# bhavyageethika/multimodal_autonomous_driving_perception_and_planning

Hardware: AMD Instinct MI355X
Metric: end-to-end frames/sec (1280x720 synthetic) (higher is better)
Workload: dtype f64; 1 GPU; config4: 64 stream(s)/GPU x 1-frame window per step, 1280x720, simulated detection + IoU tracker + 6-state KF + 21-candidate planner, one launch per step, up to 4 consecutive steps in flight; streams_per_gpu=64, window=1, graph=False, taggers=False, allgather_track_tables=False, fused_step=True, overlapped_steps=4, steps_per_library_call=8, parallelism=stream-sharded x1

## Files before the change

multimodal_autonomous_driving_perception_and_planning_amd/csrc/common.h:

```cpp
#pragma once
#include <hip/hip_runtime.h>

#include <cstdarg>
#include <cstdio>
#include <vector>

#include "avhot.h"

struct PlannerTables;

struct av_ctx {
    int device = -1;
    int n_cus = 256;
    hipStream_t side = nullptr;
    hipEvent_t ev_fork = nullptr, ev_join = nullptr;
    bool planner_ready = false;
    av_planner_cfg pcfg{};
    int n_points = 0, n_lat = 0, n_cand = 0;
    double* d_ptab = nullptr;
    double* d_cdf = nullptr;
    void* d_simtab = nullptr;
    std::vector<hipGraphExec_t> graphs;
    void* lane = nullptr;
    void* yolo = nullptr;
};

void av_set_error(const char* fmt, ...);

#define AV_HIP(expr)                                                                          \
    do {                                                                                      \
        hipError_t e_ = (expr);                                                               \
        if (e_ != hipSuccess) {                                                               \
            av_set_error("%s:%d: %s -> %s", __FILE__, __LINE__, #expr, hipGetErrorString(e_)); \
            return AV_EHIP;                                                                   \
        }                                                                                     \
    } while (0)

#define AV_REQUIRE(cond, code, ...)   \
    do {                              \
        if (!(cond)) {                \
            av_set_error(__VA_ARGS__); \
            return (code);            \
        }                             \
    } while (0)

#define AV_LAUNCH_CHECK()                                                                \
    do {                                                                                 \
        hipError_t e_ = hipGetLastError();                                               \
        if (e_ != hipSuccess) {                                                          \
            av_set_error("%s:%d: kernel launch -> %s", __FILE__, __LINE__, hipGetErrorString(e_)); \
            return AV_EHIP;                                                              \
        }                                                                                \
    } while (0)

static inline hipStream_t as_stream(av_stream_t s) { return reinterpret_cast<hipStream_t>(s); }

__device__ __forceinline__ int lane_id() { return (int)(threadIdx.x & 63); }

__device__ __forceinline__ double wave_sum(double v) {
#pragma unroll
    for (int off = 32; off > 0; off >>= 1) v += __shfl_xor(v, off, 64);
    return v;
}
template <int CTRL, int ROW_MASK = 0xF, bool BOUND = true>
__device__ __forceinline__ double dpp_mov_f64(double v) {
    const int lo = __double2loint(v), hi = __double2hiint(v);
    const int nlo = __builtin_amdgcn_update_dpp(0, lo, CTRL, ROW_MASK, 0xF, BOUND);
    const int nhi = __builtin_amdgcn_update_dpp(0, hi, CTRL, ROW_MASK, 0xF, BOUND);
    return __hiloint2double(nhi, nlo);
}
__device__ __forceinline__ double readlane_f64(double v, int l) {
    return __hiloint2double(__builtin_amdgcn_readlane(__double2hiint(v), l),
// ... 98 lines not shown
```

multimodal_autonomous_driving_perception_and_planning_amd/csrc/planner.hip:

```cpp
#include "common.h"

#include <cmath>



namespace {

struct PlanParams {
    int n, n_lat, C;
    double dt, H;
    double w_lat, w_vel, w_acc, w_curv;
    const double *t, *alpha, *q, *dtd, *lat;
    double atq[20];
};

static const double ATAN_Q[20] = {
    -0x1.5555555555549p-2, 0x1.99999999979b9p-3,  -0x1.24924923e22b4p-3, 0x1.c71c718e5a102p-4,
    -0x1.745d120df88fbp-4, 0x1.3b1362fc35ab5p-4,  -0x1.110deef367776p-4, 0x1.e1b3c8d50e91fp-5,
    -0x1.ae2c7119eb922p-5, 0x1.81fdd2525246ap-5,  -0x1.56daf4786fd80p-5, 0x1.2575526b2309ap-5,
    -0x1.d168e01adf666p-6, 0x1.462cc26bda000p-6,  -0x1.8055065b73333p-7, 0x1.693bd6b79999ap-8,
    -0x1.fdf4e15cccccdp-10, 0x1.f224118000000p-12, -0x1.2568700000000p-14, 0x1.2ed799999999ap-18,
};

__device__ __forceinline__ double atan2_fast(double y, double x, const double (&Q)[20]) {
// ... 15 lines not shown
    a = x < 0.0 ? 3.141592653589793 - a : a;
    return __builtin_copysign(a, y);
}

__host__ __device__ inline int even_up(int v) { return (v + 1) & ~1; }

__host__ __device__ inline size_t plan_lds_doubles(int G, int n, int C, int NW = 4) {
    return (size_t)G * 3 * n * 2 + even_up(G * 3 * 3) + (size_t)G * 8 + (size_t)3 * even_up(G * C) + (size_t)NW * n * 6;
}

__device__ __forceinline__ void wave_lds_fence() {
    __builtin_amdgcn_fence(__ATOMIC_RELEASE, "wavefront", "local");
    __builtin_amdgcn_wave_barrier();
    __builtin_amdgcn_fence(__ATOMIC_ACQUIRE, "wavefront", "local");
}

template <int G, int NW>
__device__ __forceinline__ void plan_block(const PlanParams& p, int f0, int n_states, const double* __restrict__ state,
                                           const double* __restrict__ ref, int n_ref, const double* __restrict__ obs, int n_obs,
                                           double* __restrict__ wp, double* __restrict__ cost, int32_t* __restrict__ order, double* sm) {
    const int n = p.n, C = p.C;
    double* vs = sm;
    double* base = vs + (size_t)G * 3 * n * 2;
    double* trig = base + even_up(G * 3 * 3);
    double* costs = trig + G * 8;
    double* stage_all = costs + 3 * even_up(G * C);
    const int CS = even_up(G * C);

    const int tid = threadIdx.x, lane = tid & 63, wid = tid >> 6;
    double* stage = stage_all + (size_t)wid * n * 6;
    constexpr int P = G * 3;
    static_assert(NW >= 2, "the heading terms take the last wave");

    auto bcast = [&](double x, int i) {
        const unsigned lo = (unsigned)__builtin_amdgcn_readlane((int)(unsigned)__double_as_longlong(x), i);
        const unsigned hi = (unsigned)__builtin_amdgcn_readlane((int)(unsigned)((unsigned long long)__double_as_longlong(x) >> 32), i);
        return __longlong_as_double((long long)(((unsigned long long)hi << 32) | lo));
    };
    auto terms = [&](double v0, double dv, int i, double& v, double& vdt, double& velt, double& acct) {
        v = v0 + dv * p.alpha[i];
        vdt = v * p.dt;
        const double e = v - 10.0;
        velt = p.w_vel * (e * e);
        acct = 0.0;
        if (i > 0) {
            const double vp = v0 + dv * p.alpha[i - 1];
            const double a = (v - vp) / p.dtd[i];
            acct = p.w_acc * (a * a);
        }
    };
    auto cost_chains = [&](double velt, double acct, unsigned long long hasm, double* b) {
        double sv = 0.0;
#pragma unroll
        for (int i = 0; i < 64; ++i)
            if (i < n) sv = sv + bcast(velt, i);
        double run = sv, sa = 0.0;
#pragma unroll
        for (int i = 1; i < 64; ++i)
            if (i < n && ((hasm >> i) & 1ull)) {
                const double term = bcast(acct, i);
                run = run + term, sa = sa + term;
            }
        if (lane == 0) b[0] = sv, b[1] = sa, b[2] = run;
    };

    const bool fast = n <= 64 && P <= NW;
    double k_velt = 0.0, k_acct = 0.0;
    unsigned long long k_has = 0;
    bool k_live = false;
    if (fast) {
        if (wid < P) {
            const int g = wid / 3, k = wid - g * 3, f = f0 + g;
            if (f < n_states) {
                const double v0 = state[(size_t)f * 4 + 3];
                const double vt = 8.0 + 2.0 * (double)k;
                const double dv = vt - v0;
                double* o = vs + ((size_t)(g * 3 + k) * n) * 2;
                double v = 0.0, vdt = 0.0;
                bool has = false;
                if (lane < n) terms(v0, dv, lane, v, vdt, k_velt, k_acct), has = lane > 0 && p.dtd[lane] > 0.0;
                k_has = __ballot(has), k_live = true;
                double sacc = 0.0, my_s = 0.0;
#pragma unroll
                for (int i = 1; i < 64; ++i)
                    if (i < n) {
                        sacc = sacc + bcast(vdt, i);
                        my_s = lane == i ? sacc : my_s;
                    }
                if (lane < n) o[2 * lane] = v, o[2 * lane + 1] = my_s;
            }
        }
    } else {
        for (int pr = wid; pr < P; pr += NW) {
            const int g = pr / 3, k = pr - g * 3, f = f0 + g;
            if (f >= n_states) continue;
            const double v0 = state[(size_t)f * 4 + 3];
            const double vt = 8.0 + 2.0 * (double)k;
            const double dv = vt - v0;
            double* o = vs + ((size_t)(g * 3 + k) * n) * 2;
            double* b = base + (g * 3 + k) * 3;
            double* tv = stage;
            for (int i = lane; i < n; i += 64) {
                double v, vdt, velt, acct;
                terms(v0, dv, i, v, vdt, velt, acct);
                o[2 * i] = v, tv[i] = vdt, tv[n + i] = velt, tv[2 * n + i] = acct;
            }
            wave_lds_fence();
            if (lane == 0) {
                double sacc = 0.0, sv = 0.0;
                o[1] = 0.0;
                sv = sv + tv[n];
                for (int i = 1; i < n; ++i) {
                    sacc = sacc + tv[i];
                    o[2 * i + 1] = sacc;
                    sv = sv + tv[n + i];
// ... 594 lines not shown
```

multimodal_autonomous_driving_perception_and_planning_amd/csrc/step.hip:

```cpp
#define AVHOT_DEVICE_ONLY
#include "simdet.hip"
#include "tracker.hip"
#include "kf.hip"
#include "planner.hip"
#undef AVHOT_DEVICE_ONLY

namespace {

struct StepArgs {
    int S, h, w, dcap, tcap;
    av_tracker_cfg tcfg;
    av_kf_cfg kcfg;
    PlanParams pp;
    int32_t* frame_count; const SimRow* tab; const double* cdf;
    int32_t *det_n, *det_box, *det_cls; double* det_conf; int32_t* det_status;
    unsigned char* trk_state; av_track_row* snap; int32_t* snap_n; int32_t* det2trk;
    const double* z; double *kf_state, *vstate, *plan_state;
    double *wp, *cost; int32_t* order;
    uint8_t* wire; int stream0, frame0;
    int* flags; int seq, spin, fence, stage_off;
};

constexpr int STEP_NW = 8;

// ... 12 lines not shown
        t = n;
    }
};

__device__ void StepClock::start(const StepArgs& a, int role) {
    on = a.flags && (a.fence & 8) && threadIdx.x == 0;
    if (!on) return;
    acc = reinterpret_cast<unsigned long long*>(a.flags + flag_stats(a.S)) + role * 16;
    t = __builtin_amdgcn_s_memrealtime();
    atomicAdd(acc + 15, 1ull);
}

__device__ __forceinline__ bool seq_enter(const StepArgs& a, int slot, int* go) {
    if (threadIdx.x == 0) {
        int ok = 0;
        int* const counter = a.flags + 32 * slot;
        int* const fault = a.flags + flag_fault(a.S);
        const int want = a.seq, spin = a.spin;
        for (int n = 0; n <= spin; ++n) {
            if ((int)((unsigned)__hip_atomic_load(counter, __ATOMIC_RELAXED, __HIP_MEMORY_SCOPE_AGENT) - (unsigned)want) >= 0) { ok = 1; break; }
            if ((n & 255) == 255 && __hip_atomic_load(fault, __ATOMIC_RELAXED, __HIP_MEMORY_SCOPE_AGENT) != 0) break;
        }
        if (!ok) atomicOr(a.flags + flag_fault(a.S), 1);
        if (ok && (a.fence & 8) && a.seq != 0) {
            const unsigned long long tp = __hip_atomic_load(reinterpret_cast<unsigned long long*>(a.flags + 32 * slot + 2), __ATOMIC_RELAXED,
                                                            __HIP_MEMORY_SCOPE_AGENT);
            const unsigned long long now = __builtin_amdgcn_s_memrealtime();
            unsigned long long* acc = reinterpret_cast<unsigned long long*>(a.flags + flag_stats(a.S)) + (slot & 1) * 16;
            if (now > tp) atomicAdd(acc + 8, now - tp), atomicAdd(acc + 9, 1ull);
        }
        *go = ok;
    }
    __syncthreads();
    if (!*go) return false;
    if (a.fence & 1) __builtin_amdgcn_fence(__ATOMIC_ACQUIRE, "agent");
    return true;
}
__device__ __forceinline__ void seq_leave(const StepArgs& a, int slot) {
    if (a.fence & 2) __builtin_amdgcn_fence(__ATOMIC_RELEASE, "agent");
    if (a.fence & 8)
        __hip_atomic_store(reinterpret_cast<unsigned long long*>(a.flags + 32 * slot + 2), __builtin_amdgcn_s_memrealtime(), __ATOMIC_RELAXED,
                           __HIP_MEMORY_SCOPE_AGENT);
    __hip_atomic_store(a.flags + 32 * slot, (int)((unsigned)a.seq + 1u), __ATOMIC_RELAXED, __HIP_MEMORY_SCOPE_AGENT);
}
__device__ __forceinline__ void fetch_record(const void* src, void* dst_lds, int n8, int first, int end, bool coherent) {
    unsigned long long* g = const_cast<unsigned long long*>(reinterpret_cast<const unsigned long long*>(src));
    unsigned long long* l = reinterpret_cast<unsigned long long*>(dst_lds);
    if ((int)threadIdx.x < first || (int)threadIdx.x >= end) return;
    for (int i = (int)threadIdx.x - first; i < n8; i += end - first)
        l[i] = coherent ? __hip_atomic_load(g + i, __ATOMIC_RELAXED, __HIP_MEMORY_SCOPE_AGENT) : g[i];
}

template <int PW>
__global__ void __launch_bounds__(PW * 64) hot_step_kernel(StepArgs a) {
    extern __shared__ __attribute__((aligned(16))) unsigned char smem[];
    __shared__ int go, fc_stage;
    __shared__ __attribute__((aligned(16))) double kf_stage[AV_KF_STATE_DOUBLES + 2];
    __shared__ __attribute__((aligned(16))) int d_box[8 * 4];
    __shared__ __attribute__((aligned(16))) double d_conf[8], d_area[8], z_stage[4];
    __shared__ int d_cls[8], d_n[1];
    const int tid = threadIdx.x;
    const bool seq = a.flags != nullptr;
    if ((int)blockIdx.x < a.S) {
        if (PW > STEP_NW && tid >= STEP_NW * 64) return;
        const int s = blockIdx.x;
        StepClock ck;
        ck.start(a, 0);
        int fc_before = 0;
        if (tid == 0) {
            fc_before = seq ? (int)((unsigned)a.flags[flag_base(a.S) + s] + (unsigned)a.seq) : a.frame_count[s];
            fc_stage = fc_before;
            simdet_frame<true>(0, 0, 0, a.h, a.w, a.dcap, &fc_stage, a.tab, a.cdf, d_n, d_box, d_cls, d_conf,
                               a.det_status ? a.det_status + s : nullptr);
            for (int i = 0; i < a.dcap; ++i)
                d_area[i] = (double)(d_box[4 * i + 2] - d_box[4 * i]) * (double)(d_box[4 * i + 3] - d_box[4 * i + 1]);
        }
        ck.mark(0);
        if (seq && !seq_enter(a, 2 * s, &go)) return;
        ck.mark(1);
        unsigned char* stage = smem + a.stage_off;
        int fc0 = 0;
        if (seq && tid == 0) fc0 = __hip_atomic_load(a.frame_count + s, __ATOMIC_RELAXED, __HIP_MEMORY_SCOPE_AGENT);
        fetch_record(a.trk_state + (size_t)s * state_bytes(a.tcap, a.tcfg.trajectory_length), stage,
                     (HDR_INTS * 4 + a.tcap * (int)sizeof(av_track_row)) / 8, 64, STEP_NW * 64, seq);
        if (tid == 0) {
            if (seq) {
                if (fc0 != fc_before) atomicOr(a.flags + flag_fault(a.S), 2);
                __hip_atomic_store(a.frame_count + s, fc_stage, __ATOMIC_RELAXED, __HIP_MEMORY_SCOPE_AGENT);
            } else {
                a.frame_count[s] = fc_stage;
            }
        }
        if (seq) __builtin_amdgcn_s_waitcnt(0x0F70);
        __syncthreads();
        ck.mark(2);
        if (tid < a.dcap) {
            reinterpret_cast<int4*>(a.det_box)[(size_t)s * a.dcap + tid] = reinterpret_cast<const int4*>(d_box)[tid];
            a.det_cls[(size_t)s * a.dcap + tid] = d_cls[tid];
            a.det_conf[(size_t)s * a.dcap + tid] = d_conf[tid];
            if (tid == 0) a.det_n[s] = d_n[0];
        }
        tracker_body<false, 8, STEP_NW>(a.tcfg, 1, a.dcap, d_n, d_box, d_cls, d_conf, a.tcap, a.trk_state, a.snap, a.snap_n,
                                        a.det2trk, 1, s, smem, 0xFEDCBA9876543210ull, stage, seq, 0,
                                        seq ? a.flags + 32 * (2 * s) : nullptr, (int)((unsigned)a.seq + 1u), (a.fence & 8) != 0, d_area);
        ck.mark(3);
        if (a.wire) {
            __syncthreads();
// ... 1 lines not shown
                wire_put(a.wire + (size_t)s * (AV_WIRE_HDR_BYTES + (size_t)a.tcap * AV_WIRE_ROW_BYTES), tid, a.snap_n[s], a.tcap,
                         a.snap + (size_t)s * a.tcap, a.stream0 + s, a.frame0 + fc_stage);
        }
    } else {
        const int s = blockIdx.x - a.S;
        StepClock ck;
        ck.start(a, 1);
        if (tid < 4) z_stage[tid] = a.z[(size_t)s * 4 + tid];
        if (seq && !seq_enter(a, 2 * s + 1, &go)) return;
        ck.mark(1);
        if (tid < 64) {
            double* rec = a.kf_state + (size_t)s * AV_KF_STATE_DOUBLES;
            fetch_record(rec, kf_stage, AV_KF_STATE_DOUBLES, 0, 64, seq);
            __builtin_amdgcn_fence(__ATOMIC_RELEASE, "workgroup", "local");
            __builtin_amdgcn_wave_barrier();
            __builtin_amdgcn_fence(__ATOMIC_ACQUIRE, "workgroup", "local");
            ck.mark(2);
            const double* z = z_stage;
            double *vs = a.vstate + (size_t)s * AV_VSTATE_DOUBLES, *ps = a.plan_state + (size_t)s * 4;
            const bool separable = kf_axis_body(a.kcfg, 1, z, nullptr, kf_stage, vs, ps, 0, tid);
            if (!separable && tid == 0) kf_dense_stream_lds(a.kcfg, 0, 1, z, nullptr, kf_stage, vs, ps);
            __builtin_amdgcn_fence(__ATOMIC_RELEASE, "workgroup", "local");
            __builtin_amdgcn_wave_barrier();
            __builtin_amdgcn_fence(__ATOMIC_ACQUIRE, "workgroup", "local");
            if (tid < AV_KF_STATE_DOUBLES) {
                if (seq)
                    __hip_atomic_store(reinterpret_cast<unsigned long long*>(rec) + tid, (unsigned long long)__double_as_longlong(kf_stage[tid]),
                                       __ATOMIC_RELAXED, __HIP_MEMORY_SCOPE_AGENT);
                else
                    rec[tid] = kf_stage[tid];
            }
        }
        ck.mark(3);
        if (seq && tid < 64) {
            __builtin_amdgcn_s_waitcnt(0x0F70);
            if (tid == 0) seq_leave(a, 2 * s + 1);
        }
        ck.mark(4);
        __syncthreads();
        plan_block<1, PW>(a.pp, s, a.S, a.plan_state, nullptr, 0, nullptr, 0, a.wp, a.cost, a.order, reinterpret_cast<double*>(smem));
        ck.mark(6);
    }
}

}

static size_t hot_step_tracker_lds(int dcap, int tcap, int& stage_off) {
    static_assert(STEP_NW == 8, "tracker_lds_bytes sizes the replica kernel's eight column waves");
    const size_t lds_t = (tracker_lds_bytes(tcap, dcap, 1, true, 0) + 15) & ~size_t(15);
    stage_off = (int)lds_t;
    return lds_t + HDR_INTS * 4 + (size_t)tcap * sizeof(av_track_row);
}

static size_t hot_step_static_lds(const void* kernel) {
    hipFuncAttributes fa{};
    return hipFuncGetAttributes(&fa, kernel) == hipSuccess ? (size_t)fa.sharedSizeBytes : (size_t)16384;
}

static int hot_step_shape(const av_ctx* ctx, int n_streams, size_t lds_t, int depth, size_t& lds_out, int& pw_out) {
    static const size_t lds_static16 = hot_step_static_lds(reinterpret_cast<const void*>(hot_step_kernel<16>));
    static const size_t lds_static8 = hot_step_static_lds(reinterpret_cast<const void*>(hot_step_kernel<8>));
    const char* pwe = getenv("AVHOT_STEP_PW");
    int pw = pwe && atoi(pwe) == 8 ? 8 : 16;
    size_t lds = 0;
    for (;;) {
        const size_t lds_p = plan_lds_doubles(1, ctx->n_points, ctx->n_cand, pw) * 8;
        lds = lds_t > lds_p ? lds_t : lds_p;
        const size_t lds_static = pw == 16 ? lds_static16 : lds_static8;
        if (lds + lds_static > 64 * 1024) {
            AV_REQUIRE(pw == 16 && !pwe, AV_EINVAL,
                       "av_hot_step: configuration needs %zu B of dynamic + %zu B of static LDS (limit 65536)", lds, lds_static);
            pw = 8;
            continue;
        }
        if (depth <= 1) break;
        int per_cu = 0;
        if (pw == 16) AV_HIP(hipOccupancyMaxActiveBlocksPerMultiprocessor(&per_cu, hot_step_kernel<16>, 16 * 64, lds));
        else AV_HIP(hipOccupancyMaxActiveBlocksPerMultiprocessor(&per_cu, hot_step_kernel<8>, 8 * 64, lds));
        if ((long long)depth * 2 * n_streams <= (long long)per_cu * ctx->n_cus) break;
        AV_REQUIRE(pw == 16 && !pwe, AV_EINVAL, "av_hot_step: %d launches of %d workgroups in flight do not fit the device (%d per CU x %d CUs)",
                   depth, 2 * n_streams, per_cu, ctx->n_cus);
        pw = 8;
    }
    lds_out = lds, pw_out = pw;
    return AV_OK;
}

static int hot_step_args(av_ctx* ctx, const av_tracker_cfg* tcfg, const av_kf_cfg* kcfg, int n_streams, int h,
                           int w, int dcap, int tcap, int32_t* frame_count, int32_t* det_n, int32_t* det_box, int32_t* det_cls,
                           double* det_conf, int32_t* det_status, void* tracker_state, av_track_row* snap, int32_t* snap_n,
                           int32_t* det2trk, const double* z, double* kf_state, double* vstate, double* plan_state,
                           double* waypoints, double* cost, int32_t* order, void* wire, int stream0, int frame0, int32_t* seq_flags,
                           int seq, StepArgs& a, size_t& lds_out, int& pw_out, int depth = 1) {
    AV_REQUIRE(ctx && tcfg && kcfg && frame_count && det_n && det_box && det_cls && det_conf && tracker_state && z && kf_state &&
                   vstate && plan_state && cost && order,
               AV_EINVAL, "av_hot_step: null argument");
    AV_REQUIRE(n_streams > 0, AV_EINVAL, "av_hot_step: n_streams must be > 0");
    AV_REQUIRE(ctx->planner_ready && ctx->d_simtab, AV_ESTATE, "av_hot_step: call av_planner_configure first");
    AV_REQUIRE((snap == nullptr) == (snap_n == nullptr), AV_EINVAL, "av_hot_step: snap and snap_n go together");
    AV_REQUIRE(!wire || snap, AV_EINVAL, "av_hot_step: the wire tables are made from the snapshot rows");
    AV_REQUIRE(tcap == 64 && dcap >= 7 && dcap <= 8 && tcfg->iou_threshold > 0.0 && tcfg->trajectory_length >= 1, AV_EINVAL,
               "av_hot_step: needs tcap 64, dcap 7..8 and iou_threshold > 0 (use the stage calls otherwise)");
    AV_REQUIRE(h > 0 && w > 121, AV_EINVAL, "av_hot_step: frame %dx%d too small", w, h);
    a = StepArgs{};
    a.S = n_streams, a.h = h, a.w = w, a.dcap = dcap, a.tcap = tcap;
    a.tcfg = *tcfg, a.kcfg = *kcfg;
    fill_params(ctx, a.pp);
    a.frame_count = frame_count, a.tab = (const SimRow*)ctx->d_simtab, a.cdf = ctx->d_cdf;
    a.det_n = det_n, a.det_box = det_box, a.det_cls = det_cls, a.det_conf = det_conf, a.det_status = det_status;
    a.trk_state = (unsigned char*)tracker_state, a.snap = snap, a.snap_n = snap_n, a.det2trk = det2trk;
    a.z = z, a.kf_state = kf_state, a.vstate = vstate, a.plan_state = plan_state;
    a.wp = waypoints, a.cost = cost, a.order = order;
    a.wire = (uint8_t*)wire, a.stream0 = stream0, a.frame0 = frame0;
    a.flags = seq_flags, a.seq = seq;
    const char* spe = seq_flags ? getenv("AVHOT_STEP_SPIN") : nullptr;
    a.spin = spe ? atoi(spe) : (1 << 22);
    const char* fe = seq_flags ? getenv("AVHOT_STEP_FENCE") : nullptr;
    a.fence = fe ? atoi(fe) : 0;
    int stage_off = 0;
    const size_t lds_t = hot_step_tracker_lds(dcap, tcap, stage_off);
    a.stage_off = stage_off;
    return hot_step_shape(ctx, n_streams, lds_t, depth, lds_out, pw_out);
}

static int hot_step_go(const StepArgs& a, size_t lds, int pw, av_stream_t stream) {
    if (pw == 16) hipLaunchKernelGGL(hot_step_kernel<16>, dim3(2 * a.S), dim3(16 * 64), lds, as_stream(stream), a);
    else hipLaunchKernelGGL(hot_step_kernel<8>, dim3(2 * a.S), dim3(8 * 64), lds, as_stream(stream), a);
    AV_LAUNCH_CHECK();
    return AV_OK;
}

static int hot_step_launch(av_ctx* ctx, av_stream_t stream, const av_tracker_cfg* tcfg, const av_kf_cfg* kcfg, int n_streams, int h,
                           int w, int dcap, int tcap, int32_t* frame_count, int32_t* det_n, int32_t* det_box, int32_t* det_cls,
                           double* det_conf, int32_t* det_status, void* tracker_state, av_track_row* snap, int32_t* snap_n,
                           int32_t* det2trk, const double* z, double* kf_state, double* vstate, double* plan_state,
                           double* waypoints, double* cost, int32_t* order, void* wire, int stream0, int frame0, int32_t* seq_flags,
                           int seq, int depth = 1) {
    StepArgs a;
    size_t lds;
    int pw;
    const int rc = hot_step_args(ctx, tcfg, kcfg, n_streams, h, w, dcap, tcap, frame_count, det_n, det_box, det_cls, det_conf, det_status,
                                 tracker_state, snap, snap_n, det2trk, z, kf_state, vstate, plan_state, waypoints, cost, order, wire, stream0,
                                 frame0, seq_flags, seq, a, lds, pw, depth);
    return rc != AV_OK ? rc : hot_step_go(a, lds, pw, stream);
}

extern "C" int av_hot_step_fits(av_ctx* ctx, int n_streams, int dcap, int tcap, int depth) {
    AV_REQUIRE(ctx && n_streams > 0 && depth >= 1, AV_EINVAL, "av_hot_step_fits: bad argument");
    AV_REQUIRE(ctx->planner_ready, AV_ESTATE, "av_hot_step_fits: call av_planner_configure first");
    AV_REQUIRE(tcap == 64 && dcap >= 7 && dcap <= 8, AV_EINVAL, "av_hot_step_fits: needs tcap 64, dcap 7..8");
    AV_HIP(hipSetDevice(ctx->device));
    int stage_off = 0;
    size_t lds = 0;
    int pw = 0;
    return hot_step_shape(ctx, n_streams, hot_step_tracker_lds(dcap, tcap, stage_off), depth, lds, pw);
}

extern "C" int av_hot_step(av_ctx* ctx, av_stream_t stream, const av_tracker_cfg* tcfg, const av_kf_cfg* kcfg, int n_streams, int h,
                           int w, int dcap, int tcap, int32_t* frame_count, int32_t* det_n, int32_t* det_box, int32_t* det_cls,
                           double* det_conf, int32_t* det_status, void* tracker_state, av_track_row* snap, int32_t* snap_n,
                           int32_t* det2trk, const double* z, double* kf_state, double* vstate, double* plan_state,
                           double* waypoints, double* cost, int32_t* order, void* wire, int stream0, int frame0) {
    return hot_step_launch(ctx, stream, tcfg, kcfg, n_streams, h, w, dcap, tcap, frame_count, det_n, det_box, det_cls, det_conf, det_status,
                           tracker_state, snap, snap_n, det2trk, z, kf_state, vstate, plan_state, waypoints, cost, order, wire, stream0,
                           frame0, nullptr, 0);
}

extern "C" int av_hot_step_seq(av_ctx* ctx, av_stream_t stream, const av_tracker_cfg* tcfg, const av_kf_cfg* kcfg, int n_streams, int h,
                               int w, int dcap, int tcap, int32_t* frame_count, int32_t* det_n, int32_t* det_box, int32_t* det_cls,
                               double* det_conf, int32_t* det_status, void* tracker_state, av_track_row* snap, int32_t* snap_n,
                               int32_t* det2trk, const double* z, double* kf_state, double* vstate, double* plan_state,
                               double* waypoints, double* cost, int32_t* order, void* wire, int stream0, int frame0,
                               int32_t* seq_flags, int seq, int depth) {
    AV_REQUIRE(seq_flags, AV_EINVAL, "av_hot_step_seq: needs the sequence flags (AV_STEP_FLAG_INTS(n_streams) int32)");
    AV_REQUIRE(depth >= 2 && depth <= AV_STEP_MAX_DEPTH, AV_EINVAL, "av_hot_step_seq: depth %d not in [2, %d]", depth, AV_STEP_MAX_DEPTH);
    return hot_step_launch(ctx, stream, tcfg, kcfg, n_streams, h, w, dcap, tcap, frame_count, det_n, det_box, det_cls, det_conf, det_status,
                           tracker_state, snap, snap_n, det2trk, z, kf_state, vstate, plan_state, waypoints, cost, order, wire, stream0,
                           frame0, seq_flags, seq, depth);
}

extern "C" int av_hot_steps_seq(av_ctx* ctx, int depth, const av_stream_t* streams, const av_tracker_cfg* tcfg, const av_kf_cfg* kcfg,
                                int n_streams, int h, int w, int dcap, int tcap, int32_t* frame_count, int32_t* det_status,
                                void* tracker_state, double* kf_state, const av_step_set* sets, const double* z_steps, void* wire_steps,
                                int stream0, int frame0, int32_t* seq_flags, int seq0, int n_steps) {
    AV_REQUIRE(seq_flags && n_steps > 0 && sets && streams, AV_EINVAL, "av_hot_steps_seq: bad argument");
    AV_REQUIRE(depth >= 2 && depth <= AV_STEP_MAX_DEPTH, AV_EINVAL, "av_hot_steps_seq: depth %d not in [2, %d]", depth, AV_STEP_MAX_DEPTH);
    for (int k = 0; k < depth; ++k)
        for (int j = 0; j < k; ++j)
            AV_REQUIRE(streams[k] != streams[j], AV_EINVAL, "av_hot_steps_seq: the %d steps in flight need %d different HIP streams", depth, depth);
    StepArgs par[AV_STEP_MAX_DEPTH];
    size_t lds = 0;
    int pw = 16;
    for (int k = 0; k < depth; ++k) {
        const av_step_set& b = sets[k];
        const int rc = hot_step_args(ctx, tcfg, kcfg, n_streams, h, w, dcap, tcap, frame_count, b.det_n, b.det_box, b.det_cls, b.det_conf, det_status,
                                     tracker_state, b.snap, b.snap_n, b.det2trk, z_steps ? z_steps : b.z, kf_state, b.vstate, b.plan_state,
                                     b.waypoints, b.cost, b.order, wire_steps, stream0, frame0, seq_flags, seq0, par[k], lds, pw, depth);
        if (rc != AV_OK) return rc;
    }
    const size_t zb = (size_t)n_streams * 4, wb = (size_t)n_streams * (AV_WIRE_HDR_BYTES + (size_t)tcap * AV_WIRE_ROW_BYTES);
    for (int i = 0; i < n_steps; ++i) {
        const int q = (int)((unsigned)seq0 + (unsigned)i), k = (int)((unsigned)q % (unsigned)depth);
        StepArgs& a = par[k];
        a.seq = q;
        if (z_steps) a.z = z_steps + (size_t)i * zb;
        if (wire_steps) a.wire = (uint8_t*)wire_steps + (size_t)i * wb;
        const int rc = hot_step_go(a, lds, pw, streams[k]);
        if (rc != AV_OK) return rc;
    }
    return AV_OK;
}
```

multimodal_autonomous_driving_perception_and_planning_amd/pipeline.py:

```python
import ctypes as C

import numpy as np
import torch

from . import _native as nat


class HotLoop:
    def __init__(self, n_streams=1, window=1, h=720, w=1280, tcap=64, dcap=8, device=0,
                 tracker_kw=None, kf_kw=None, planner_kw=None, keep_waypoints=True, keep_snapshots=True,
                 ctx=None, fused_step=None, overlap=1):
        if not torch.cuda.is_available():
            raise RuntimeError("HotLoop needs a HIP device; this package has no CPU path")
        self.S, self.W, self.h, self.w, self.tcap, self.dcap = n_streams, window, h, w, tcap, dcap
        self.dev = torch.device("cuda", device)
        self.ctx = ctx or nat.Context(device)
        self.L = nat.lib()
        tk = dict(iou_threshold=0.3, max_age=30, min_hits=3, trajectory_length=50)
        tk.update(tracker_kw or {})
        self.tcfg = nat.TrackerCfg(**tk)
        kk = dict(dt=0.033, process_noise=0.1, measurement_noise=1.0)
        kk.update(kf_kw or {})
        self.kcfg = nat.KfCfg(**kk)
        pk = dict(planning_horizon=5.0, dt=0.1, num_samples=7, w_lateral=1.0, w_velocity=0.5,
# ... 4 lines not shown
        n, c = C.c_int(), C.c_int()
        nat.check(self.L.av_planner_dims(self.ctx.handle, C.byref(n), C.byref(c)))
        self.n_points, self.n_cand = n.value, c.value

        S, W, d = n_streams, window, self.dev
        i32, f64 = torch.int32, torch.float64
        self.frame_count = torch.zeros(S, dtype=i32, device=d)
        self.det_n = torch.zeros(S, W, dtype=i32, device=d)
        self.det_box = torch.zeros(S, W, dcap, 4, dtype=i32, device=d)
        self.det_cls = torch.zeros(S, W, dcap, dtype=i32, device=d)
        self.det_conf = torch.zeros(S, W, dcap, dtype=f64, device=d)
        self.det_status = torch.zeros(S, dtype=i32, device=d)
        self.trk_bytes = int(self.L.av_tracker_state_bytes(tcap, self.tcfg.trajectory_length))
        self.trk_state = torch.zeros(S, self.trk_bytes, dtype=torch.uint8, device=d)
        self.keep_snapshots = keep_snapshots
        self.snap = torch.zeros(S, W, tcap, nat.TRACK_ROW_BYTES, dtype=torch.uint8, device=d) if keep_snapshots else None
        self.snap_n = torch.zeros(S, W, dtype=i32, device=d) if keep_snapshots else None
        self.det2trk = torch.zeros(S, W, dcap, dtype=i32, device=d)
        self.z = torch.zeros(S, W, 4, dtype=f64, device=d)
        self.kf_state = torch.zeros(S, nat.KF_STATE_DOUBLES, dtype=f64, device=d)
        self.vstate = torch.zeros(S, W, nat.VSTATE_DOUBLES, dtype=f64, device=d)
        self.plan_state = torch.zeros(S, W, 4, dtype=f64, device=d)
        self.keep_waypoints = keep_waypoints
        self.wp = (torch.zeros(S * W, self.n_cand, self.n_points, nat.WP_DOUBLES, dtype=f64, device=d)
                   if keep_waypoints else None)
        self.cost = torch.zeros(S * W, self.n_cand, dtype=f64, device=d)
        self.order = torch.zeros(S * W, self.n_cand, dtype=i32, device=d)
        self.stream = torch.cuda.Stream(device=d)
        self.graph_id = None
        self._graphs = {}
        can_fuse = window == 1 and tcap == 64 and 7 <= dcap <= 8 and self.tcfg.iou_threshold > 0
        if fused_step and not can_fuse:
            raise ValueError("fused_step needs window 1, tcap 64, dcap 7..8 and iou_threshold > 0")
        if can_fuse and fused_step is not False:
            rc = self.L.av_hot_step_fits(self.ctx.handle, S, dcap, tcap, 1)
            if rc != 0:
                if fused_step:
                    raise ValueError("fused_step: %s" % self.L.av_last_error_string().decode())
                can_fuse = False
        self.fused_step = can_fuse if fused_step is None else bool(fused_step)
        self.wire = None
        self._wire_ids = (0, 0)
        self.overlap = int(overlap)
        if self.overlap not in (1, 2, 3, 4):
            raise ValueError("overlap is 1 .. 4")
        if self.overlap > 1:
            if not self.fused_step:
                raise ValueError("overlap=2 needs the fused step (window 1, tcap 64, dcap 7..8, iou_threshold > 0)")
            names = [k for k in self._PER_STEP if getattr(self, k) is not None]
            self._sets = [{k: getattr(self, k) for k in names}] + [{k: torch.zeros_like(getattr(self, k)) for k in names}
                                                                   for _ in range(self.overlap - 1)]
            self._pstreams = [self.stream] + [torch.cuda.Stream(device=d) for _ in range(self.overlap - 1)]
            self.seq_flags = torch.zeros(nat.step_flag_ints(S), dtype=i32, device=d)
            self._seq, self._stepped = 0, False
            self._csets = None
            self.reset()
            try:
                self._enqueue_step_seq()
                self.synchronize()
            except RuntimeError as e:
                raise ValueError("overlap=%d: %s" % (self.overlap, e)) from None
        self.reset()

    _PER_STEP = ("det_n", "det_box", "det_cls", "det_conf", "snap", "snap_n", "det2trk", "z", "vstate", "plan_state", "wp",
                 "cost", "order")

    @property
    def _s(self):
        return C.c_void_p(self.stream.cuda_stream)

    _i32 = staticmethod(nat.step_i32)

    def _serial_only(self, what):
        if self.overlap != 1:
            raise RuntimeError("%s is not available with overlap=2.. (only the one-launch step is ordered across the loop's streams)" % what)

    def reset(self, frame_offsets=None):
        h, L = self.ctx.handle, self.L
        if self.overlap > 1:
            for st in self._pstreams:
                st.synchronize()
        nat.check(L.av_tracker_reset(h, self._s, self.S, self.tcap, self.tcfg.trajectory_length, nat.ptr(self.trk_state)))
        nat.check(L.av_kf_reset(h, self._s, self.S, nat.ptr(self.kf_state)))
        with torch.cuda.stream(self.stream):
            if frame_offsets is None:
                self.frame_count.zero_()
            else:
                self.frame_count.copy_(torch.as_tensor(np.asarray(frame_offsets, np.int32)), non_blocking=False)
            if self.overlap > 1:
                self.seq_flags.zero_()
                self.seq_flags[64 * self.S + 32:65 * self.S + 32].copy_(self.frame_count)
        if self.overlap > 1:
            self._seq, self._stepped = 0, False
            self.__dict__.update(self._sets[0])
        self.stream.synchronize()

    def load_measurements(self, z, all_sets=False):
        if self.overlap > 1:
            zt = torch.as_tensor(np.ascontiguousarray(z, np.float64)).view(self.S, self.W, 4)
            for k in (range(self.overlap) if all_sets else (self._seq % self.overlap,)):
                with torch.cuda.stream(self._pstreams[k]):
                    self._sets[k]["z"].copy_(zt)
                self._pstreams[k].synchronize()
            self.z = self._sets[self._seq % self.overlap]["z"]
            return
        with torch.cuda.stream(self.stream):
# ... 71 lines not shown
                                      self._bev_cap, nat.ptr(self._bev_n)))
        nat.check(self.L.av_raster_draw(self.ctx.handle, st, self.S, self._bev_cfg.height, self._bev_cfg.width, nat.ptr(self.bev),
                                        nat.ptr(self._bev_prims), self._bev_cap, nat.ptr(self._bev_n), None, 0))

    def enqueue_plan(self, stream=None):
        self._serial_only("enqueue_plan")
        nat.check(self.L.av_planner_plan(self.ctx.handle, stream or self._s, self.S * self.W,
                                         nat.ptr(self.plan_state), None, 0, None, 0, nat.ptr(self.wp),
                                         nat.ptr(self.cost), nat.ptr(self.order)))

    def set_wire(self, wire, stream0=0, frame0=0):
        if wire is not None and not (self.fused_step and self.keep_snapshots):
            raise RuntimeError("set_wire needs the fused step and keep_snapshots=True")
        self.wire, self._wire_ids = wire, (int(stream0), int(frame0))

    def enqueue_step_fused(self, stream=None):
        if self.overlap > 1:
            return self._enqueue_step_seq(stream)
        nat.check(self.L.av_hot_step(self.ctx.handle, stream or self._s, C.byref(self.tcfg), C.byref(self.kcfg), self.S, self.h,
                                     self.w, self.dcap, self.tcap, nat.ptr(self.frame_count), nat.ptr(self.det_n),
                                     nat.ptr(self.det_box), nat.ptr(self.det_cls), nat.ptr(self.det_conf),
                                     nat.ptr(self.det_status), nat.ptr(self.trk_state), nat.ptr(self.snap), nat.ptr(self.snap_n),
                                     nat.ptr(self.det2trk), nat.ptr(self.z), nat.ptr(self.kf_state), nat.ptr(self.vstate),
                                     nat.ptr(self.plan_state), nat.ptr(self.wp), nat.ptr(self.cost), nat.ptr(self.order),
                                     nat.ptr(self.wire), self._wire_ids[0], self._wire_ids[1]))

    def _enqueue_step_seq(self, stream=None):
        if stream is not None:
            raise RuntimeError("overlap=2.. launches on the loop's own streams")
        k = self._seq % self.overlap
        b = self._sets[k]
        self.__dict__.update(b)
        nat.check(self.L.av_hot_step_seq(self.ctx.handle, C.c_void_p(self._pstreams[k].cuda_stream), C.byref(self.tcfg), C.byref(self.kcfg),
                                         self.S, self.h, self.w, self.dcap, self.tcap, nat.ptr(self.frame_count), nat.ptr(b["det_n"]),
                                         nat.ptr(b["det_box"]), nat.ptr(b["det_cls"]), nat.ptr(b["det_conf"]),
                                         nat.ptr(self.det_status), nat.ptr(self.trk_state), nat.ptr(b.get("snap")), nat.ptr(b.get("snap_n")),
                                         nat.ptr(b["det2trk"]), nat.ptr(b["z"]), nat.ptr(self.kf_state), nat.ptr(b["vstate"]),
                                         nat.ptr(b["plan_state"]), nat.ptr(b.get("wp")), nat.ptr(b["cost"]), nat.ptr(b["order"]),
                                         nat.ptr(self.wire), self._wire_ids[0], self._wire_ids[1], nat.ptr(self.seq_flags), self._i32(self._seq), self.overlap))
        self._seq = (self._seq + 1) & 0xFFFFFFFF
        self._stepped = True

    def enqueue_steps(self, n_steps, z_steps=None, wire_steps=None):
        if self.overlap < 2:
            raise RuntimeError("enqueue_steps needs overlap=2..")
        if n_steps <= 0:
            return
        if self._csets is None:
            def cset(b):
                m = {"wp": "waypoints"}
                return nat.StepSet(**{m.get(k, k): (b[k].data_ptr() if b.get(k) is not None else None) for k in self._PER_STEP})
            self._csets = (nat.StepSet * self.overlap)(*[cset(b) for b in self._sets])
            self._cstreams = (C.c_void_p * self.overlap)(*[st.cuda_stream for st in self._pstreams])
        if z_steps is not None and (z_steps.dtype != torch.float64 or z_steps.numel() != n_steps * self.S * 4 or not z_steps.is_contiguous()):
            raise ValueError("z_steps: contiguous float64 [n_steps, S, 4]")
        if wire_steps is not None:
            wb = int(self.L.av_wire_table_bytes(self.tcap))
            if not (self.keep_snapshots and wire_steps.dtype == torch.uint8 and wire_steps.numel() == n_steps * self.S * wb and wire_steps.is_contiguous()):
                raise ValueError("wire_steps: contiguous uint8 [n_steps, S, %d] (and keep_snapshots=True)" % wb)
        nat.check(self.L.av_hot_steps_seq(self.ctx.handle, self.overlap, self._cstreams,
                                          C.byref(self.tcfg), C.byref(self.kcfg), self.S, self.h, self.w, self.dcap, self.tcap,
                                          nat.ptr(self.frame_count), nat.ptr(self.det_status), nat.ptr(self.trk_state), nat.ptr(self.kf_state),
                                          self._csets, nat.ptr(z_steps), nat.ptr(wire_steps),
                                          self._wire_ids[0], self._wire_ids[1], nat.ptr(self.seq_flags), self._i32(self._seq), int(n_steps)))
        self._seq = (self._seq + int(n_steps)) & 0xFFFFFFFF
        self._stepped = True
        self.__dict__.update(self._sets[((self._seq - 1) & 0xFFFFFFFF) % self.overlap])

    def tune_streams(self, pool=8, candidates=12, steps=600):
        import time
        if self.overlap < 2:
            return []
        self.synchronize(check=False)
        D = self.overlap
        fresh = [torch.cuda.Stream(device=self.dev) for _ in range(max(pool, D))]
        rs = np.random.RandomState(12345)
        sets = [list(self._pstreams)] + [fresh[i:i + D] for i in range(0, len(fresh) - D + 1, D)]
        while len(sets) < candidates:
            sets.append([fresh[i] for i in sorted(rs.choice(len(fresh), D, replace=False))])
        tried = []
        for cand in sets:
            self._pstreams, self.stream = list(cand), cand[0]
            self._csets = None
            self.reset()
            self.enqueue_steps(64)
            self.synchronize()
            t0 = time.perf_counter()
            self.enqueue_steps(steps)
            self.synchronize()
            tried.append(((time.perf_counter() - t0) / steps * 1e6, cand))
        best = min(tried, key=lambda x: x[0])
        self._pstreams, self.stream = list(best[1]), best[1][0]
        self._csets = None
        self.reset()
        return [round(t, 2) for t, _ in tried]

    def step_stream(self):
        return self._pstreams[((self._seq - 1) & 0xFFFFFFFF) % self.overlap] if self.overlap > 1 and self._stepped else self.stream

    def enqueue_step(self):
        if self.fused_step:
            return self.enqueue_step_fused()
        h, L, s = self.ctx.handle, self.L, self._s
        nat.check(L.av_fork(h, s))
        self.enqueue_detect(self.ctx.side_stream)
        self.enqueue_track(self.ctx.side_stream)
        self.enqueue_kf()
        self.enqueue_plan()
        nat.check(L.av_join(h, s))

    def capture(self):
        self._serial_only("capture()")
        gid = C.c_int(-1)
        nat.check(self.L.av_graph_begin(self.ctx.handle, self._s))
        try:
            self.enqueue_step()
        finally:
# ... 241 lines not shown
```

Before: 12.73 million frames/s.

## Cache step launch plan, add 12-wave kernel shape, trim host arg marshalling

Caches the per-depth launch shape (LDS size, waves per block) in the context so that occupancy queries, env lookups and attribute queries are not repeated on every library call. It also validates only the per-step pointer sets for later in-flight slots instead of rebuilding full args each time. A new 12-wave kernel variant with a min-blocks launch bound is added as an intermediate fallback shape, and the planner cost loop now exits early instead of masking. On the Python side the constant ctypes argument tuple is prebuilt. The cache key could go stale if other context state changes, and the new 12-wave shape only matters when the 16-wave shape does not fit.

```diff
diff --git a/multimodal_autonomous_driving_perception_and_planning_amd/csrc/common.h b/multimodal_autonomous_driving_perception_and_planning_amd/csrc/common.h
--- a/multimodal_autonomous_driving_perception_and_planning_amd/csrc/common.h
+++ b/multimodal_autonomous_driving_perception_and_planning_amd/csrc/common.h
@@ -9,6 +9,13 @@
 
 struct PlannerTables;
 
+struct av_step_plan {
+    bool valid = false;
+    int n_streams = 0, dcap = 0, tcap = 0, n_points = 0, n_cand = 0, pw_hook = 0;
+    size_t lds = 0;
+    int pw = 0, stage_off = 0;
+};
+
 struct av_ctx {
     int device = -1;
     int n_cus = 256;
@@ -18,6 +25,7 @@
     av_planner_cfg pcfg{};
     int n_points = 0, n_lat = 0, n_cand = 0;
     double* d_ptab = nullptr;
+    av_step_plan step_plan[AV_STEP_MAX_DEPTH];
     double* d_cdf = nullptr;
     void* d_simtab = nullptr;
     std::vector<hipGraphExec_t> graphs;
diff --git a/multimodal_autonomous_driving_perception_and_planning_amd/csrc/planner.hip b/multimodal_autonomous_driving_perception_and_planning_amd/csrc/planner.hip
--- a/multimodal_autonomous_driving_perception_and_planning_amd/csrc/planner.hip
+++ b/multimodal_autonomous_driving_perception_and_planning_amd/csrc/planner.hip
@@ -91,15 +91,19 @@
     auto cost_chains = [&](double velt, double acct, unsigned long long hasm, double* b) {
         double sv = 0.0;
 #pragma unroll
-        for (int i = 0; i < 64; ++i)
-            if (i < n) sv = sv + bcast(velt, i);
+        for (int i = 0; i < 64; ++i) {
+            if (i >= n) break;
+            sv = sv + bcast(velt, i);
+        }
         double run = sv, sa = 0.0;
 #pragma unroll
-        for (int i = 1; i < 64; ++i)
-            if (i < n && ((hasm >> i) & 1ull)) {
+        for (int i = 1; i < 64; ++i) {
+            if (i >= n) break;
+            if ((hasm >> i) & 1ull) {
                 const double term = bcast(acct, i);
                 run = run + term, sa = sa + term;
             }
+        }
         if (lane == 0) b[0] = sv, b[1] = sa, b[2] = run;
     };
 
diff --git a/multimodal_autonomous_driving_perception_and_planning_amd/csrc/step.hip b/multimodal_autonomous_driving_perception_and_planning_amd/csrc/step.hip
--- a/multimodal_autonomous_driving_perception_and_planning_amd/csrc/step.hip
+++ b/multimodal_autonomous_driving_perception_and_planning_amd/csrc/step.hip
@@ -88,7 +88,7 @@
 }
 
 template <int PW>
-__global__ void __launch_bounds__(PW * 64) hot_step_kernel(StepArgs a) {
+__global__ void __launch_bounds__(PW * 64, PW == 12 ? 6 : 1) hot_step_kernel(StepArgs a) {
     extern __shared__ __attribute__((aligned(16))) unsigned char smem[];
     __shared__ int go, fc_stage;
     __shared__ __attribute__((aligned(16))) double kf_stage[AV_KF_STATE_DOUBLES + 2];
@@ -196,37 +196,86 @@
     return lds_t + HDR_INTS * 4 + (size_t)tcap * sizeof(av_track_row);
 }
 
-static size_t hot_step_static_lds(const void* kernel) {
-    hipFuncAttributes fa{};
-    return hipFuncGetAttributes(&fa, kernel) == hipSuccess ? (size_t)fa.sharedSizeBytes : (size_t)16384;
-}
-
-static int hot_step_shape(const av_ctx* ctx, int n_streams, size_t lds_t, int depth, size_t& lds_out, int& pw_out) {
-    static const size_t lds_static16 = hot_step_static_lds(reinterpret_cast<const void*>(hot_step_kernel<16>));
-    static const size_t lds_static8 = hot_step_static_lds(reinterpret_cast<const void*>(hot_step_kernel<8>));
-    const char* pwe = getenv("AVHOT_STEP_PW");
-    int pw = pwe && atoi(pwe) == 8 ? 8 : 16;
-    size_t lds = 0;
-    for (;;) {
+static const void* hot_step_fn(int pw) {
+    return pw == 16 ? reinterpret_cast<const void*>(hot_step_kernel<16>)
+                    : pw == 12 ? reinterpret_cast<const void*>(hot_step_kernel<12>) : reinterpret_cast<const void*>(hot_step_kernel<8>);
+}
+
+static size_t hot_step_static_lds(int pw) {
+    auto ask = [](int w) {
+        hipFuncAttributes fa{};
+        return hipFuncGetAttributes(&fa, hot_step_fn(w)) == hipSuccess ? (size_t)fa.sharedSizeBytes : (size_t)16384;
+    };
+    static const size_t lds16 = ask(16), lds12 = ask(12), lds8 = ask(8);
+    return pw == 16 ? lds16 : pw == 12 ? lds12 : lds8;
+}
+
+struct StepHooks { int pw; bool pw_forced; int spin, fence; };
+static StepHooks read_step_hooks(bool seq) {
+    StepHooks hk{0, false, 1 << 22, 0};
+    if (const char* e = getenv("AVHOT_STEP_PW")) {
+        const int v = atoi(e);
+        hk.pw = v == 8 || v == 12 ? v : 16, hk.pw_forced = true;
+    }
+    if (seq) {
+        if (const char* e = getenv("AVHOT_STEP_SPIN")) hk.spin = atoi(e);
+        if (const char* e = getenv("AVHOT_STEP_FENCE")) hk.fence = atoi(e);
+    }
+    return hk;
+}
+
+static int hot_step_shape(const av_ctx* ctx, int n_streams, size_t lds_t, int depth, const StepHooks& hk, size_t& lds_out, int& pw_out) {
+    static const int shapes[3] = {16, 12, 8};
+    for (int pw : shapes) {
+        if (hk.pw_forced && pw != hk.pw) continue;
+        const bool last = hk.pw_forced || pw == 8;
         const size_t lds_p = plan_lds_doubles(1, ctx->n_points, ctx->n_cand, pw) * 8;
-        lds = lds_t > lds_p ? lds_t : lds_p;
-        const size_t lds_static = pw == 16 ? lds_static16 : lds_static8;
+        const size_t lds = lds_t > lds_p ? lds_t : lds_p, lds_static = hot_step_static_lds(pw);
         if (lds + lds_static > 64 * 1024) {
-            AV_REQUIRE(pw == 16 && !pwe, AV_EINVAL,
-                       "av_hot_step: configuration needs %zu B of dynamic + %zu B of static LDS (limit 65536)", lds, lds_static);
-            pw = 8;
+            AV_REQUIRE(!last, AV_EINVAL, "av_hot_step: configuration needs %zu B of dynamic + %zu B of static LDS (limit 65536)", lds,
+                       lds_static);
             continue;
         }
-        if (depth <= 1) break;
-        int per_cu = 0;
-        if (pw == 16) AV_HIP(hipOccupancyMaxActiveBlocksPerMultiprocessor(&per_cu, hot_step_kernel<16>, 16 * 64, lds));
-        else AV_HIP(hipOccupancyMaxActiveBlocksPerMultiprocessor(&per_cu, hot_step_kernel<8>, 8 * 64, lds));
-        if ((long long)depth * 2 * n_streams <= (long long)per_cu * ctx->n_cus) break;
-        AV_REQUIRE(pw == 16 && !pwe, AV_EINVAL, "av_hot_step: %d launches of %d workgroups in flight do not fit the device (%d per CU x %d CUs)",
-                   depth, 2 * n_streams, per_cu, ctx->n_cus);
-        pw = 8;
-    }
-    lds_out = lds, pw_out = pw;
+        if (depth > 1) {
+            int per_cu = 0;
+            AV_HIP(hipOccupancyMaxActiveBlocksPerMultiprocessor(&per_cu, hot_step_fn(pw), pw * 64, lds));
+            if ((long long)depth * 2 * n_streams > (long long)per_cu * ctx->n_cus) {
+                AV_REQUIRE(!last, AV_EINVAL, "av_hot_step: %d launches of %d workgroups in flight do not fit the device (%d per CU x %d CUs)",
+                           depth, 2 * n_streams, per_cu, ctx->n_cus);
+                continue;
+            }
+        }
+        lds_out = lds, pw_out = pw;
+        return AV_OK;
+    }
+    return AV_EINVAL;
+}
+
+static int hot_step_plan(av_ctx* ctx, int n_streams, int dcap, int tcap, int depth, const StepHooks& hk, av_step_plan& out) {
+    av_step_plan* slot = depth >= 1 && depth <= AV_STEP_MAX_DEPTH ? &ctx->step_plan[depth - 1] : nullptr;
+    if (slot && slot->valid && slot->n_streams == n_streams && slot->dcap == dcap && slot->tcap == tcap &&
+        slot->n_points == ctx->n_points && slot->n_cand == ctx->n_cand && slot->pw_hook == hk.pw) {
+        out = *slot;
+        return AV_OK;
+    }
+    av_step_plan p;
+    p.n_streams = n_streams, p.dcap = dcap, p.tcap = tcap, p.n_points = ctx->n_points, p.n_cand = ctx->n_cand, p.pw_hook = hk.pw;
+    const size_t lds_t = hot_step_tracker_lds(dcap, tcap, p.stage_off);
+    const int rc = hot_step_shape(ctx, n_streams, lds_t, depth, hk, p.lds, p.pw);
+    if (rc != AV_OK) return rc;
+    p.valid = true;
+    if (slot) *slot = p;
+    out = p;
+    return AV_OK;
+}
+
+static int check_step_set(const int32_t* det_n, const int32_t* det_box, const int32_t* det_cls, const double* det_conf,
+                          const av_track_row* snap, const int32_t* snap_n, const double* z, const double* vstate, const double* plan_state,
+                          const double* cost, const int32_t* order, const void* wire) {
+    AV_REQUIRE(det_n && det_box && det_cls && det_conf && z && vstate && plan_state && cost && order, AV_EINVAL,
+               "av_hot_step: null argument");
+    AV_REQUIRE((snap == nullptr) == (snap_n == nullptr), AV_EINVAL, "av_hot_step: snap and snap_n go together");
+    AV_REQUIRE(!wire || snap, AV_EINVAL, "av_hot_step: the wire tables are made from the snapshot rows");
     return AV_OK;
 }
 
@@ -235,17 +284,20 @@
                            double* det_conf, int32_t* det_status, void* tracker_state, av_track_row* snap, int32_t* snap_n,
                            int32_t* det2trk, const double* z, double* kf_state, double* vstate, double* plan_state,
                            double* waypoints, double* cost, int32_t* order, void* wire, int stream0, int frame0, int32_t* seq_flags,
-                           int seq, StepArgs& a, size_t& lds_out, int& pw_out, int depth = 1) {
-    AV_REQUIRE(ctx && tcfg && kcfg && frame_count && det_n && det_box && det_cls && det_conf && tracker_state && z && kf_state &&
-                   vstate && plan_state && cost && order,
-               AV_EINVAL, "av_hot_step: null argument");
+                           int seq, StepArgs& a, av_step_plan& plan, int depth = 1) {
+    AV_REQUIRE(ctx && tcfg && kcfg && frame_count && tracker_state && kf_state, AV_EINVAL, "av_hot_step: null argument");
     AV_REQUIRE(n_streams > 0, AV_EINVAL, "av_hot_step: n_streams must be > 0");
     AV_REQUIRE(ctx->planner_ready && ctx->d_simtab, AV_ESTATE, "av_hot_step: call av_planner_configure first");
-    AV_REQUIRE((snap == nullptr) == (snap_n == nullptr), AV_EINVAL, "av_hot_step: snap and snap_n go together");
-    AV_REQUIRE(!wire || snap, AV_EINVAL, "av_hot_step: the wire tables are made from the snapshot rows");
+    {
+        const int rc = check_step_set(det_n, det_box, det_cls, det_conf, snap, snap_n, z, vstate, plan_state, cost, order, wire);
+        if (rc != AV_OK) return rc;
+    }
     AV_REQUIRE(tcap == 64 && dcap >= 7 && dcap <= 8 && tcfg->iou_threshold > 0.0 && tcfg->trajectory_length >= 1, AV_EINVAL,
                "av_hot_step: needs tcap 64, dcap 7..8 and iou_threshold > 0 (use the stage calls otherwise)");
     AV_REQUIRE(h > 0 && w > 121, AV_EINVAL, "av_hot_step: frame %dx%d too small", w, h);
+    const StepHooks hk = read_step_hooks(seq_flags != nullptr);
+    const int rc = hot_step_plan(ctx, n_streams, dcap, tcap, depth, hk, plan);
+    if (rc != AV_OK) return rc;
     a = StepArgs{};
     a.S = n_streams, a.h = h, a.w = w, a.dcap = dcap, a.tcap = tcap;
     a.tcfg = *tcfg, a.kcfg = *kcfg;
@@ -257,19 +309,16 @@
     a.wp = waypoints, a.cost = cost, a.order = order;
     a.wire = (uint8_t*)wire, a.stream0 = stream0, a.frame0 = frame0;
     a.flags = seq_flags, a.seq = seq;
-    const char* spe = seq_flags ? getenv("AVHOT_STEP_SPIN") : nullptr;
-    a.spin = spe ? atoi(spe) : (1 << 22);
-    const char* fe = seq_flags ? getenv("AVHOT_STEP_FENCE") : nullptr;
-    a.fence = fe ? atoi(fe) : 0;
-    int stage_off = 0;
-    const size_t lds_t = hot_step_tracker_lds(dcap, tcap, stage_off);
-    a.stage_off = stage_off;
-    return hot_step_shape(ctx, n_streams, lds_t, depth, lds_out, pw_out);
-}
-
-static int hot_step_go(const StepArgs& a, size_t lds, int pw, av_stream_t stream) {
-    if (pw == 16) hipLaunchKernelGGL(hot_step_kernel<16>, dim3(2 * a.S), dim3(16 * 64), lds, as_stream(stream), a);
-    else hipLaunchKernelGGL(hot_step_kernel<8>, dim3(2 * a.S), dim3(8 * 64), lds, as_stream(stream), a);
+    a.spin = hk.spin, a.fence = hk.fence;
+    a.stage_off = plan.stage_off;
+    return AV_OK;
+}
+
+static int hot_step_go(const StepArgs& a, const av_step_plan& plan, av_stream_t stream) {
+    const dim3 grid(2 * a.S), block(plan.pw * 64);
+    if (plan.pw == 16) hipLaunchKernelGGL(hot_step_kernel<16>, grid, block, plan.lds, as_stream(stream), a);
+    else if (plan.pw == 12) hipLaunchKernelGGL(hot_step_kernel<12>, grid, block, plan.lds, as_stream(stream), a);
+    else hipLaunchKernelGGL(hot_step_kernel<8>, grid, block, plan.lds, as_stream(stream), a);
     AV_LAUNCH_CHECK();
     return AV_OK;
 }
@@ -281,12 +330,11 @@
                            double* waypoints, double* cost, int32_t* order, void* wire, int stream0, int frame0, int32_t* seq_flags,
                            int seq, int depth = 1) {
     StepArgs a;
-    size_t lds;
-    int pw;
+    av_step_plan plan;
     const int rc = hot_step_args(ctx, tcfg, kcfg, n_streams, h, w, dcap, tcap, frame_count, det_n, det_box, det_cls, det_conf, det_status,
                                  tracker_state, snap, snap_n, det2trk, z, kf_state, vstate, plan_state, waypoints, cost, order, wire, stream0,
-                                 frame0, seq_flags, seq, a, lds, pw, depth);
-    return rc != AV_OK ? rc : hot_step_go(a, lds, pw, stream);
+                                 frame0, seq_flags, seq, a, plan, depth);
+    return rc != AV_OK ? rc : hot_step_go(a, plan, stream);
 }
 
 extern "C" int av_hot_step_fits(av_ctx* ctx, int n_streams, int dcap, int tcap, int depth) {
@@ -294,10 +342,8 @@
     AV_REQUIRE(ctx->planner_ready, AV_ESTATE, "av_hot_step_fits: call av_planner_configure first");
     AV_REQUIRE(tcap == 64 && dcap >= 7 && dcap <= 8, AV_EINVAL, "av_hot_step_fits: needs tcap 64, dcap 7..8");
     AV_HIP(hipSetDevice(ctx->device));
-    int stage_off = 0;
-    size_t lds = 0;
-    int pw = 0;
-    return hot_step_shape(ctx, n_streams, hot_step_tracker_lds(dcap, tcap, stage_off), depth, lds, pw);
+    av_step_plan plan;
+    return hot_step_plan(ctx, n_streams, dcap, tcap, depth, read_step_hooks(false), plan);
 }
 
 extern "C" int av_hot_step(av_ctx* ctx, av_stream_t stream, const av_tracker_cfg* tcfg, const av_kf_cfg* kcfg, int n_streams, int h,
@@ -333,14 +379,25 @@
         for (int j = 0; j < k; ++j)
             AV_REQUIRE(streams[k] != streams[j], AV_EINVAL, "av_hot_steps_seq: the %d steps in flight need %d different HIP streams", depth, depth);
     StepArgs par[AV_STEP_MAX_DEPTH];
-    size_t lds = 0;
-    int pw = 16;
-    for (int k = 0; k < depth; ++k) {
-        const av_step_set& b = sets[k];
+    av_step_plan plan;
+    {
+        const av_step_set& b = sets[0];
         const int rc = hot_step_args(ctx, tcfg, kcfg, n_streams, h, w, dcap, tcap, frame_count, b.det_n, b.det_box, b.det_cls, b.det_conf, det_status,
                                      tracker_state, b.snap, b.snap_n, b.det2trk, z_steps ? z_steps : b.z, kf_state, b.vstate, b.plan_state,
-                                     b.waypoints, b.cost, b.order, wire_steps, stream0, frame0, seq_flags, seq0, par[k], lds, pw, depth);
+                                     b.waypoints, b.cost, b.order, wire_steps, stream0, frame0, seq_flags, seq0, par[0], plan, depth);
         if (rc != AV_OK) return rc;
+    }
+    for (int k = 1; k < depth; ++k) {
+        const av_step_set& b = sets[k];
+        const int rc = check_step_set(b.det_n, b.det_box, b.det_cls, b.det_conf, b.snap, b.snap_n, z_steps ? z_steps : b.z, b.vstate,
+                                      b.plan_state, b.cost, b.order, wire_steps);
+        if (rc != AV_OK) return rc;
+        StepArgs& a = par[k];
+        a = par[0];
+        a.det_n = b.det_n, a.det_box = b.det_box, a.det_cls = b.det_cls, a.det_conf = b.det_conf;
+        a.snap = b.snap, a.snap_n = b.snap_n, a.det2trk = b.det2trk;
+        if (!z_steps) a.z = b.z;
+        a.vstate = b.vstate, a.plan_state = b.plan_state, a.wp = b.waypoints, a.cost = b.cost, a.order = b.order;
     }
     const size_t zb = (size_t)n_streams * 4, wb = (size_t)n_streams * (AV_WIRE_HDR_BYTES + (size_t)tcap * AV_WIRE_ROW_BYTES);
     for (int i = 0; i < n_steps; ++i) {
@@ -349,7 +406,7 @@
         a.seq = q;
         if (z_steps) a.z = z_steps + (size_t)i * zb;
         if (wire_steps) a.wire = (uint8_t*)wire_steps + (size_t)i * wb;
-        const int rc = hot_step_go(a, lds, pw, streams[k]);
+        const int rc = hot_step_go(a, plan, streams[k]);
         if (rc != AV_OK) return rc;
     }
     return AV_OK;
diff --git a/multimodal_autonomous_driving_perception_and_planning_amd/pipeline.py b/multimodal_autonomous_driving_perception_and_planning_amd/pipeline.py
--- a/multimodal_autonomous_driving_perception_and_planning_amd/pipeline.py
+++ b/multimodal_autonomous_driving_perception_and_planning_amd/pipeline.py
@@ -80,6 +80,7 @@
                                                                    for _ in range(self.overlap - 1)]
             self._pstreams = [self.stream] + [torch.cuda.Stream(device=d) for _ in range(self.overlap - 1)]
             self.seq_flags = torch.zeros(nat.step_flag_ints(S), dtype=i32, device=d)
+            self._seq_flags_ptr = nat.ptr(self.seq_flags)
             self._seq, self._stepped = 0, False
             self._csets = None
             self.reset()
@@ -257,17 +258,17 @@
                 return nat.StepSet(**{m.get(k, k): (b[k].data_ptr() if b.get(k) is not None else None) for k in self._PER_STEP})
             self._csets = (nat.StepSet * self.overlap)(*[cset(b) for b in self._sets])
             self._cstreams = (C.c_void_p * self.overlap)(*[st.cuda_stream for st in self._pstreams])
+            self._cargs = (self.ctx.handle, self.overlap, self._cstreams, C.byref(self.tcfg), C.byref(self.kcfg), self.S, self.h,
+                           self.w, self.dcap, self.tcap, nat.ptr(self.frame_count), nat.ptr(self.det_status),
+                           nat.ptr(self.trk_state), nat.ptr(self.kf_state), self._csets)
         if z_steps is not None and (z_steps.dtype != torch.float64 or z_steps.numel() != n_steps * self.S * 4 or not z_steps.is_contiguous()):
             raise ValueError("z_steps: contiguous float64 [n_steps, S, 4]")
         if wire_steps is not None:
             wb = int(self.L.av_wire_table_bytes(self.tcap))
             if not (self.keep_snapshots and wire_steps.dtype == torch.uint8 and wire_steps.numel() == n_steps * self.S * wb and wire_steps.is_contiguous()):
                 raise ValueError("wire_steps: contiguous uint8 [n_steps, S, %d] (and keep_snapshots=True)" % wb)
-        nat.check(self.L.av_hot_steps_seq(self.ctx.handle, self.overlap, self._cstreams,
-                                          C.byref(self.tcfg), C.byref(self.kcfg), self.S, self.h, self.w, self.dcap, self.tcap,
-                                          nat.ptr(self.frame_count), nat.ptr(self.det_status), nat.ptr(self.trk_state), nat.ptr(self.kf_state),
-                                          self._csets, nat.ptr(z_steps), nat.ptr(wire_steps),
-                                          self._wire_ids[0], self._wire_ids[1], nat.ptr(self.seq_flags), self._i32(self._seq), int(n_steps)))
+        nat.check(self.L.av_hot_steps_seq(*self._cargs, nat.ptr(z_steps), nat.ptr(wire_steps),
+                                          self._wire_ids[0], self._wire_ids[1], self._seq_flags_ptr, self._i32(self._seq), int(n_steps)))
         self._seq = (self._seq + int(n_steps)) & 0xFFFFFFFF
         self._stepped = True
         self.__dict__.update(self._sets[((self._seq - 1) & 0xFFFFFFFF) % self.overlap])
```

Result: faster. 13.40 million frames/s, median of 6 (+5.3%).
